# ai4ce/DiscoNet

Measured on AMD Instinct MI355X. Metric: scenes/sec (5-agent 256x256 BEV), higher is better.
Workload: dtype f16 hi+lo pair per value (32 bits; 22-bit significand for |x| >= 0.125, f16 exponent range, lo subnormal below: absolute floor 2^-25); conv products as split-f16 x3 MFMA, f32 accumulate; 1 GPU; DiscoNet det eval forward (--com disco), 5-agent, batch 4 per GPU, 256x256x13 BEV, no KD, sparse voxel lists -> dense -> enc -> DiscoGraph fusion -> dec -> cls/reg heads; agents=5, batch_per_gpu=4, conv_math=sp, launch=hipGraph replay, parallelism=scene-parallel x1 (no data-path collective)

## Files before the change

disconet_amd/csrc/build.py:

```python
import glob
import hashlib
import os
import subprocess
import sys
from concurrent.futures import ThreadPoolExecutor

HERE = os.path.dirname(os.path.abspath(__file__))
ROOT = os.path.dirname(os.path.dirname(HERE))
SOURCES = ["common.hip", "conv_mfma.hip", "conv_sp.hip", "conv_spq.hip", "voxel.hip", "warp.hip", "fuse_reduce.hip", "fuse_tail.hip", "fuse_mlp.hip", "agent_fuse.hip", "decode.hip", "detect.hip", "ap_match.hip", "assign.hip", "track.hip", "mot_eval.hip", "idf_eval.hip", "hota_eval.hip",
           "conv_wgrad.hip", "train_ops.hip", "seg_ops.hip", "seg_eval.hip", "render.hip", "lidar.hip"]
FLAGS = ["--offload-arch=gfx950", "-O3", "-std=c++17", "-fPIC", "-Wno-comment"]
LIB_PATH = os.path.join(os.path.dirname(HERE), "libdisconet_hip.so")


def tree_files():
    files = []
    for pat in ("*.hip", "*.inl", "*.h"):
        files += glob.glob(os.path.join(HERE, pat))
    files += glob.glob(os.path.join(ROOT, "include", "*.h"))
    return sorted(os.path.relpath(f, ROOT) for f in files)


def sources_present():
    return all(os.path.exists(os.path.join(HERE, s)) for s in SOURCES)


_HASH_CACHE = {}


def tree_hash(extra_flags=(), unit=None):
    try:
        stamp = (tuple(extra_flags), unit, tuple((rel,) + tuple(os.stat(os.path.join(ROOT, rel))[k] for k in (6, 8))
                                                  for rel in tree_files()))
    except OSError:
        stamp = None
    if stamp is not None and stamp in _HASH_CACHE:
        return _HASH_CACHE[stamp]
    h = hashlib.sha256()
    h.update(" ".join(FLAGS + list(extra_flags)).encode())
    for rel in tree_files():
        if unit is not None and rel.endswith(".hip") and os.path.basename(rel) != unit:
            continue
        h.update(b"\0" + rel.encode() + b"\0")
        with open(os.path.join(ROOT, rel), "rb") as f:
            h.update(f.read())
    if stamp is not None:
        _HASH_CACHE[stamp] = h.hexdigest()[:16]
    return h.hexdigest()[:16]


def built_id(path=None):
    import re
    path = path or LIB_PATH
    if not os.path.exists(path):
        return None
    with open(path, "rb") as f:
        m = re.search(rb"dn-build-id:([0-9a-f]{16})", f.read())
    return m.group(1).decode() if m else None


def needs_build():
    return built_id() != tree_hash()
# ... 62 lines not shown
```

disconet_amd/csrc/common.hip:

```cpp
#include "dn_internal.h"

namespace dn {
char* err_buf() {
  static thread_local char buf[512] = {0};
  return buf;
}
namespace {
typedef unsigned u32x4 __attribute__((ext_vector_type(4)));
__global__ void __launch_bounds__(256) zero_fill_kernel(unsigned char* p, size_t head, size_t vecs, size_t tail) {
  const size_t tid = blockIdx.x * (size_t)blockDim.x + threadIdx.x, stride = (size_t)gridDim.x * blockDim.x;
  if (tid < head) p[tid] = 0;
  u32x4* v = reinterpret_cast<u32x4*>(p + head);
  for (size_t i = tid; i < vecs; i += stride) v[i] = u32x4{0u, 0u, 0u, 0u};
  if (tid < tail) p[head + 16 * vecs + tid] = 0;
}
}

hipError_t zero_fill(void* ptr, size_t bytes, hipStream_t stream) {
  if (bytes == 0) return hipSuccess;
  unsigned char* p = static_cast<unsigned char*>(ptr);
  size_t head = (16 - (reinterpret_cast<size_t>(p) & 15)) & 15;
  if (head > bytes) head = bytes;
  const size_t vecs = (bytes - head) / 16, tail = bytes - head - 16 * vecs;
  const size_t want = (vecs + 255) / 256;
  const int blocks = (int)(want < 1 ? 1 : (want > 8192 ? 8192 : want));
  hipLaunchKernelGGL(zero_fill_kernel, dim3(blocks), dim3(256), 0, stream, p, head, vecs, tail);
  return hipGetLastError();
}
}

extern "C" int dn_version(void) { return 153; }

#ifndef DN_BUILD_ID
#error "build through disconet_amd/csrc/build.py (it passes -DDN_BUILD_ID)"
#endif
static const char dn_build_id_marker[] = "dn-build-id:" DN_BUILD_ID;
extern "C" const char* dn_build_id(void) { return dn_build_id_marker + 12; }

extern "C" int dn_sp_range_flags_async(unsigned* dst_device, int reset, void* stream) {
  DN_REQUIRE(dst_device != nullptr, "sp_range_flags_async: null destination");
  hipStream_t s = (hipStream_t)stream;
  if ((reset & 2) && dn::zero_fill(dst_device, sizeof(unsigned), s) != hipSuccess)
    return dn::fail(DN_ERR_LAUNCH, "sp_range_flags_async: zero fill of the destination failed");
  const bool clear = (reset & 1) != 0;
  dn::range_collect_conv_sp(dst_device, clear, s);
  dn::range_collect_conv_spq(dst_device, clear, s);
  dn::range_collect_fuse_mlp(dst_device, clear, s);
  dn::range_collect_conv_wgrad(dst_device, clear, s);
  return dn::check_launch("sp_range_collect_kernel");
}

extern "C" unsigned dn_sp_range_flags(int reset) {
  unsigned* d = nullptr;
  unsigned v = 0;
  if (hipDeviceSynchronize() != hipSuccess || hipMalloc((void**)&d, sizeof v) != hipSuccess) return 0x80000000u;
  bool ok = hipMemcpy(d, &v, sizeof v, hipMemcpyHostToDevice) == hipSuccess &&
            dn_sp_range_flags_async(d, reset ? 1 : 0, nullptr) == DN_OK &&
            hipMemcpy(&v, d, sizeof v, hipMemcpyDeviceToHost) == hipSuccess;
  (void)hipFree(d);
  return ok ? v : 0x80000000u;
}

extern "C" const char* dn_last_error(void) { return dn::err_buf(); }
```

disconet_amd/csrc/conv_sp.hip:

```cpp
#ifndef DN_PHASE_TIMING
#define DN_PHASE_TIMING 0
#endif
#ifndef DN_SP_ABL
#define DN_SP_ABL 0
#endif
#include "dn_internal.h"
#include "sp_layout.h"
#include "sp_device.h"
#include "sp_split.h"
#include <array>
#include <cstdlib>
#include <type_traits>
#include <utility>

#if DN_PHASE_TIMING
__device__ unsigned long long g_phase_cycles[8];
extern "C" int dn_sp_phase_cycles(unsigned long long* host8, int reset) {
  if (hipDeviceSynchronize() != hipSuccess) return -1;
  if (host8 && hipMemcpyFromSymbol(host8, HIP_SYMBOL(g_phase_cycles), sizeof(unsigned long long) * 8) != hipSuccess) return -1;
  if (reset) { unsigned long long z[8] = {0}; if (hipMemcpyToSymbol(HIP_SYMBOL(g_phase_cycles), z, sizeof z) != hipSuccess) return -1; }
  return 0;
}
#endif

// ... 1116 lines not shown
}

inline int out_dim(int in, int ksize, int stride) {
  const int pad = ksize / 2;
  return (in + 2 * pad - ksize) / stride + 1;
}
inline int cout_pad_of(int c_out) { return (c_out + 63) / 64 * 64; }
using sp::chunks_of;
int g_sp_upmode = -1;
inline int up_mode(const dn_conv_desc& d) {
  const int mode = g_sp_upmode >= 0 ? g_sp_upmode : 2;
  const bool ok = d.up0 == 1 && d.ksize == 3 && d.stride == 1 && d.c0 > 0 && d.c0 % 16 == 0 && d.h_in % 2 == 0 &&
                  d.w_in % 2 == 0;
  return ok ? (mode < 0 ? 0 : mode > 2 ? 2 : mode) : 0;
}
inline bool up_merged(const dn_conv_desc& d) { return up_mode(d) == 1; }
inline size_t packed_blocks(const dn_conv_desc& d);
inline int packed_chunks(const dn_conv_desc& d) { return (chunks_of(d.c0) + chunks_of(d.c1) + 3) / 4 * 4; }

int validate(const dn_conv_desc* d) {
  DN_REQUIRE(d != nullptr, "spconv: null descriptor");
  DN_REQUIRE(d->ksize == 1 || d->ksize == 3, "spconv: ksize %d unsupported (1 or 3)", d->ksize);
  DN_REQUIRE(d->stride == 1 || (d->stride == 2 && d->ksize == 3),
             "spconv: stride %d with ksize %d unsupported", d->stride, d->ksize);
  DN_REQUIRE(d->n_images > 0 && d->h_in > 0 && d->w_in > 0, "spconv: empty input");
  DN_REQUIRE(d->c0 > 0 && d->c1 >= 0 && d->c_out > 0, "spconv: bad channel counts");
  DN_REQUIRE(d->up0 == 0 || d->up0 == 1, "spconv: up0 must be 0 or 1");
  DN_REQUIRE(d->math != 3 || (d->ksize == 3 && d->stride == 1 && d->c1 == 0 && d->up0 == 0),
             "spconv: a hi-only source 0 (math = 3) needs a 3x3 stride-1 single-source layer");
  DN_REQUIRE(d->math != 4 || (d->ksize == 3 && d->stride == 1 && d->c1 == 0 && d->up0 == 0 && d->c0 <= 32),
             "spconv: a bit-grid source 0 (math = 4) needs a 3x3 stride-1 single-source layer of <= 32 channels");
  DN_REQUIRE(!d->up0 || (d->h_in % 2 == 0 && d->w_in % 2 == 0), "spconv: x2-upsampled source needs even h_in/w_in");
  DN_REQUIRE(d->c1 == 0 || (d->c0 % 16 == 0 && d->ksize == 3), "spconv: concat needs 3x3 and c0 %% 16 == 0 (c0 = %d)", d->c0);
  const size_t hs0 = d->up0 ? d->h_in / 2 : d->h_in, ws0 = d->up0 ? d->w_in / 2 : d->w_in;
  DN_REQUIRE(hs0 * ws0 * chunks_of(d->c0) * 64 < (1ull << 31) &&
                 (size_t)d->h_in * d->w_in * chunks_of(d->c1) * 64 < (1ull << 31),
             "spconv: one image must stay below 2 GiB");
  return DN_OK;
}

inline size_t packed_blocks(const dn_conv_desc& d) {
  const int nch = packed_chunks(d);
  if (up_mode(d) == 2) return dn::spq_packed_blocks(chunks_of(d.c0), nch);
  if (up_merged(d)) return (size_t)chunks_of(d.c0) * 12 + (size_t)(nch - chunks_of(d.c0)) * 9;
  return (size_t)nch * d.ksize * d.ksize;
}

enum SpCfgId { S3_256x64, S3_256x32, S3_128x64, S3_64x64, S3S2_128x64, S3S2_64x64, S1_256x64, S1_64x64,
               S3_256x64_T9, S3_512x64, S3_256x128, S1_256x64_C1, S3_256x32_ST, S3_64x64_T9, S3_128x64_T9,
               S3S2_64x64_T9, S3S2_128x64_T9, SP_CFG_COUNT };
enum SpForceId {
  FORCE_SPQ_BN32 = 20, FORCE_SPQ_BN64 = 21, FORCE_SPQ_DEEP = 22,
  FORCE_SPQ_ABL = 22,
  FORCE_TOOLS = 100,
  FORCE_ABL_256x64 = 100, FORCE_ABL_256x32 = 200,
  FORCE_ABL_64x64_T9 = 300,
  FORCE_ABL_S2_64x64 = 400,
};

template <int KS_, int STRIDE_, int TH_, int TW_, int BN_, int TG_, int CA_, int WAVES_M_, int WAVES_N_, int WTM_, int WTN_>
struct Geom {
  using G = Geom;
  static constexpr int KS = KS_, STRIDE = STRIDE_, TH = TH_, TW = TW_, BN = BN_, TG = TG_, CA = CA_, WAVES_M = WAVES_M_,
                       WAVES_N = WAVES_N_, WTM = WTM_, WTN = WTN_;
};
template <SpCfgId ID> struct Tile;
#define SP_TILE(id, bias_, deep_, ...) \
  template <> struct Tile<id> : __VA_ARGS__ { static constexpr float bias = bias_; static constexpr SpCfgId deep = deep_; }
SP_TILE(S3_256x64,      1.00f, S3_256x64_T9,   Geom<3, 1, 8,  32, 64,  3, 1, 4, 1, 2, 2>);
SP_TILE(S3_256x32,      1.15f, S3_256x32,      Geom<3, 1, 8,  32, 32,  3, 1, 4, 1, 2, 1>);
SP_TILE(S3_128x64,      1.10f, S3_128x64_T9,   Geom<3, 1, 8,  16, 64,  3, 1, 2, 2, 2, 1>);
SP_TILE(S3_64x64,       1.40f, S3_64x64_T9,    Geom<3, 1, 8,  8,  64,  3, 1, 2, 2, 1, 1>);
SP_TILE(S3S2_128x64,    1.45f, S3S2_128x64_T9, Geom<3, 2, 8,  16, 64,  3, 1, 2, 2, 2, 1>);
SP_TILE(S3S2_64x64,     1.00f, S3S2_64x64_T9,  Geom<3, 2, 8,  8,  64,  3, 1, 2, 2, 1, 1>);
SP_TILE(S1_256x64,      1.00f, S1_256x64,      Geom<1, 1, 8,  32, 64,  1, 2, 4, 1, 2, 2>);
SP_TILE(S1_64x64,       1.30f, S1_64x64,       Geom<1, 1, 8,  8,  64,  1, 4, 2, 2, 1, 1>);
SP_TILE(S3_256x64_T9,   1.f,   S3_256x64_T9,   Geom<3, 1, 8,  32, 64,  9, 1, 4, 1, 2, 2>);
SP_TILE(S3_512x64,      1.f,   S3_512x64,      Geom<3, 1, 16, 32, 64,  3, 1, 8, 1, 2, 2>);
SP_TILE(S3_256x128,     1.f,   S3_256x128,     Geom<3, 1, 8,  32, 128, 3, 1, 4, 2, 2, 2>);
SP_TILE(S1_256x64_C1,   1.2f,  S1_256x64_C1,   Geom<1, 1, 8,  32, 64,  1, 1, 4, 1, 2, 2>);
SP_TILE(S3_256x32_ST,   1.f,   S3_256x32_ST,   Tile<S3_256x32>::G);
SP_TILE(S3_64x64_T9,    1.f,   S3_64x64_T9,    Geom<3, 1, 8,  8,  64,  9, 1, 2, 2, 1, 1>);
SP_TILE(S3_128x64_T9,   1.f,   S3_128x64_T9,   Geom<3, 1, 8,  16, 64,  9, 1, 2, 2, 2, 1>);
SP_TILE(S3S2_64x64_T9,  1.f,   S3S2_64x64_T9,  Geom<3, 2, 8,  8,  64,  9, 1, 2, 2, 1, 1>);
SP_TILE(S3S2_128x64_T9, 1.f,   S3S2_128x64_T9, Geom<3, 2, 8,  16, 64,  9, 1, 2, 2, 2, 1>);
#undef SP_TILE

struct SpCfg { SpCfgId id; int th, tw, bn, ca; float bias; SpCfgId deep; };
template <int... I>
constexpr std::array<SpCfg, sizeof...(I)> sp_cfgs(std::integer_sequence<int, I...>) {
  return {{{(SpCfgId)I, Tile<(SpCfgId)I>::TH, Tile<(SpCfgId)I>::TW, Tile<(SpCfgId)I>::BN, Tile<(SpCfgId)I>::CA,
            Tile<(SpCfgId)I>::bias, Tile<(SpCfgId)I>::deep}...}};
}
constexpr std::array<SpCfg, SP_CFG_COUNT> kSpCfgs = sp_cfgs(std::make_integer_sequence<int, SP_CFG_COUNT>{});
int g_sp_force = -1;

SpCfg select_cfg(const dn_conv_desc& d, int kslices = 1, bool can_split = false) {
  const int ho = out_dim(d.h_in, d.ksize, d.stride), wo = out_dim(d.w_in, d.ksize, d.stride);
  static const SpCfgId c3[] = {S3_256x64, S3_256x32, S3_128x64, S3_64x64};
  static const SpCfgId c3s2[] = {S3S2_128x64, S3S2_64x64};
  static const SpCfgId c1[] = {S1_256x64, S1_64x64, S1_256x64_C1};
  static const SpCfgId c3up[] = {S3_256x32, S3_128x64};
  const bool upm = up_merged(d);
  static const SpCfgId c3ks[] = {S3_256x32, S3_128x64, S3_64x64};
  const bool ksl = kslices > 1 && d.ksize == 3 && !upm;
  const SpCfgId* cand = d.ksize == 1 ? c1 : (d.stride == 2 ? c3s2 : (upm ? c3up : (ksl ? c3ks : c3)));
// ... 369 lines not shown

extern "C" int dn_spconv2d_nhwc(const dn_conv_desc* d, const void* src0, const void* src1, const void* packed,
                                const float* scale, const float* shift, float* out_nhwc, int ld_nhwc, void* stream) {
  DN_REQUIRE(d && out_nhwc && ld_nhwc >= d->c_out && ld_nhwc % 4 == 0 && d->c_out % 4 == 0 &&
                 (reinterpret_cast<uintptr_t>(out_nhwc) & 15) == 0,
             "spconv nhwc: the fp32 NHWC output needs c_out %% 4 == 0, ld >= c_out, ld %% 4 == 0, 16-byte alignment");
  return spconv2d_impl(d, src0, src1, packed, scale, shift, nullptr, out_nhwc, ld_nhwc, stream);
}

inline bool ks_layer(const dn_conv_desc& d) { return d.ksize == 3 && d.math != 3 && d.math != 4 && up_mode(d) != 1; }

extern "C" int dn_spconv_ks_supported(const dn_conv_desc* d, int kslices) {
  if (validate(d) != DN_OK) return 0;
  if (kslices == 1) return 1;
  if (kslices != 2 && kslices != 4) return 0;
  return ks_layer(*d) && chunks_of(d->c0) + chunks_of(d->c1) >= kslices ? 1 : 0;
}

extern "C" size_t dn_spconv_workspace_bytes(const dn_conv_desc* d, int kslices) {
  if (validate(d) != DN_OK || kslices <= 1 || !ks_layer(*d)) return 0;
  const size_t ho = out_dim(d->h_in, d->ksize, d->stride), wo = out_dim(d->w_in, d->ksize, d->stride);
  return (size_t)kslices * d->n_images * ((ho + 7) / 8 * 8) * ((wo + 31) / 32 * 32) * ((d->c_out + 63) / 64 * 64) * sizeof(float);
}

extern "C" int dn_spconv2d_ks(const dn_conv_desc* d, int kslices, const void* src0, const void* src1, const void* packed,
                              const float* scale, const float* shift, void* out, float* out_nhwc, int ld_nhwc,
                              void* workspace, size_t workspace_bytes, void* stream) {
  DN_REQUIRE(kslices == 1 || kslices == 2 || kslices == 4, "spconv: kslices must be 1, 2 or 4 (got %d)", kslices);
  DN_REQUIRE(workspace == nullptr || (reinterpret_cast<uintptr_t>(workspace) & 15) == 0, "spconv: workspace must be 16-byte aligned");
  DN_REQUIRE(!out_nhwc || (d && ld_nhwc >= d->c_out && ld_nhwc % 4 == 0 && d->c_out % 4 == 0 &&
                           (reinterpret_cast<uintptr_t>(out_nhwc) & 15) == 0),
             "spconv: the fp32 NHWC output needs c_out %% 4 == 0, ld >= c_out, ld %% 4 == 0, 16-byte alignment");
  return spconv2d_impl(d, src0, src1, packed, scale, shift, out, out_nhwc, ld_nhwc, stream, kslices, workspace, workspace_bytes);
}

namespace {
int spconv2d_impl(const dn_conv_desc* d, const void* src0, const void* src1, const void* packed, const float* scale,
                  const float* shift, void* out, float* out_nhwc, int ld_nhwc, void* stream, int kslices,
                  void* workspace, size_t workspace_bytes) {
  if (int rc = validate(d)) return rc;
  DN_REQUIRE(src0 && packed && scale && shift && (out || out_nhwc), "spconv: null pointer");
  DN_REQUIRE(d->c1 == 0 || src1, "spconv: c1 > 0 but src1 is null");
  SpArgs a;
  if (int rc = fill_args(d, src0, src1, packed, scale, shift, out, a)) return rc;
  a.out_b = out_nhwc; a.ldo_b = ld_nhwc;
  DN_REQUIRE(!out_nhwc || g_sp_force < FORCE_TOOLS, "spconv dual: not with a forced tools configuration");
  hipStream_t s = (hipStream_t)stream;
  DN_REQUIRE(kslices == 1 || (ks_layer(*d) && a.c0g + a.c1g >= kslices),
             "spconv: %d K slices need a 3x3 layer of at least that many 16-channel chunks", kslices);
  if (up_mode(*d) == 2) {
    DN_REQUIRE(a.c1g == 0 || d->c0 % 16 == 0, "spconv: concat needs c0 %% 16 == 0");
    const int f = g_sp_force;
    const int bn = f == FORCE_SPQ_BN32 ? 32 : f == FORCE_SPQ_BN64 ? 64 : f == FORCE_SPQ_DEEP ? 33 :
                   (f > FORCE_SPQ_ABL && f <= FORCE_SPQ_ABL + 3) ? 100 + (f - FORCE_SPQ_ABL) : 0;
    return dn::spq_conv(d, src0, src1, packed, (size_t)a.wpk_bytes, scale, shift, out, a.cout_pad, bn, s, kslices,
                        (float*)workspace, workspace_bytes, out_nhwc, ld_nhwc);
  }
  if (kslices > 1) {
    a.ks.count = kslices;
    a.ks.partial = (float*)workspace;
    a.ks_ws_bytes = workspace_bytes;
    const SpCfg c = select_cfg(*d, kslices, workspace != nullptr && workspace_bytes > 0);
    const int rc = launch_form<KSliced, S3_256x32, S3_128x64, S3_64x64, S3S2_128x64, S3S2_64x64, S3_64x64_T9, S3_128x64_T9,
                               S3S2_64x64_T9, S3S2_128x64_T9>(c.id, a, *d, s);
    return rc != kNotListed ? rc : dn::fail(DN_ERR_UNSUPPORTED, "spconv: tile configuration %d has no K-sliced form", (int)c.id);
  }
  if (d->math == 3) {
    if (fits_stationary<HiOnlyStationary, S3_256x32>(*d, 0, 2)) return launch_form<HiOnlyStationary, S3_256x32>(a, *d, s);
    return launch_form<HiOnly, S3_256x32>(a, *d, s);
  }
  if (d->math == 4) {
    if (fits_stationary<BitGrid, S3_256x32>(*d, 0, 2)) return launch_form<BitGrid, S3_256x32>(a, *d, s);
    return dn::fail(DN_ERR_UNSUPPORTED, "spconv: a bit-grid source needs a layer whose weights fit the LDS (c_out <= 32)");
  }
  const SpCfg c = select_cfg(*d);
  if (up_merged(*d)) {
    const int rc = launch_form<RowMerged, S3_256x64, S3_256x32, S3_128x64>(c.id, a, *d, s);
    return rc != kNotListed ? rc : dn::fail(DN_ERR_UNSUPPORTED, "spconv: tile configuration %d has no row-merged form", (int)c.id);
  }
  if (d->ksize == 3 && d->stride == 1) {
    const int rc = launch_ablation<S3_64x64_T9, 1, 2, 3, 4, 5>(g_sp_force - FORCE_ABL_64x64_T9, a, *d, s);
    if (rc != kNotListed) return rc;
  }
#if DN_SP_ABL
  if (d->ksize == 3 && d->stride == 1) {
    int rc = launch_ablation<S3_256x64, 1, 2, 3, 4, 5>(g_sp_force - FORCE_ABL_256x64, a, *d, s);
    if (rc == kNotListed) rc = launch_ablation<S3_256x32, 1, 2, 3, 4, 5, 6, 7>(g_sp_force - FORCE_ABL_256x32, a, *d, s);
    if (rc != kNotListed) return rc;
  }
  if (d->ksize == 3 && d->stride == 2) {
    if (g_sp_force == FORCE_ABL_S2_64x64) return launch_form<Plain, S3S2_64x64>(a, *d, s);
    const int rc = launch_ablation<S3S2_64x64, 1, 2, 3, 4, 5, 7>(g_sp_force - FORCE_ABL_S2_64x64, a, *d, s);
    if (rc != kNotListed) return rc;
  }
#endif
  if (g_sp_force < 0 && c.id == S3_256x32 && fits_stationary<Stationary, S3_256x32>(*d, 0, 2))
    return launch_form<Stationary, S3_256x32>(a, *d, s);
  if (g_sp_force == S3_256x32_ST) return launch_form<Stationary, S3_256x32_ST>(a, *d, s);
  static const int b3_env = [] { const char* e = getenv("DN_SP_B3"); return e ? atoi(e) : 3; }();
  if (g_sp_force < 0 && c.id == S3S2_64x64 && (b3_env & 1)) return launch_form<ThreeStages, S3S2_64x64>(a, *d, s);
  if (g_sp_force < 0 && c.id == S3_64x64 && (b3_env & 2)) return launch_form<ThreeStages, S3_64x64>(a, *d, s);
  const int rc = launch_form<Plain, S3_256x64, S3_256x32, S3_128x64, S3_64x64, S3S2_128x64, S3S2_64x64, S1_256x64, S1_64x64,
                             S3_256x64_T9, S3_512x64, S3_256x128, S1_256x64_C1, S3_64x64_T9, S3_128x64_T9, S3S2_64x64_T9,
                             S3S2_128x64_T9>(c.id, a, *d, s);
  return rc != kNotListed ? rc : dn::fail(DN_ERR_UNSUPPORTED, "spconv: no tile configuration");
}
// ... 44 lines not shown
```

disconet_amd/csrc/conv_spq.hip:

```cpp
#ifndef DN_SP_ABL
#define DN_SP_ABL 0
#endif
#include "dn_internal.h"
#include "sp_layout.h"
#include "sp_device.h"
#include "sp_split.h"
#include <type_traits>

namespace {

constexpr int kCUs = 256;

constexpr int QTH = 8, QTW = 32, QPH = QTH + 2, QPW = QTW + 2, QHALF = QPW / 2, QPITCH = QPW, QNPIX = QPH * QPITCH;
constexpr int QNW = 4, QNT = QNW * 64;
constexpr int QA_PIECES = 4 * QNPIX;
constexpr int QA_INSTR = (QA_PIECES + 63) / 64;
constexpr int QA_IT = (QA_INSTR + QNW - 1) / QNW;
constexpr int QA_STAGE = QA_INSTR * 1024;
static_assert(QA_INSTR == 22 && QA_IT == 6, "patch stage: 22 instructions, waves 0 / 1 issue 6, waves 2 / 3 issue 5");

struct SpqArgs {
  const unsigned char* src0;
  const unsigned char* src1;
  const unsigned char* wpk;
// ... 636 lines not shown
    form.grid = (int)(work > resident ? resident : work); form.total_items = (int)work;
    form.n_whole = k.n_whole; form.n_split = k.n_split;
    form.fixup_grid = k.n_split ? (int)(k.n_split > 2 * kCUs ? 2 * kCUs : k.n_split) : 0;
    dn::g_sp_last_form = form;
    hipLaunchKernelGGL(kern, dim3((unsigned)(work > resident ? resident : work)), dim3(QNT), T::LDS_BYTES, stream, a);
    if (k.n_split) {
      k.fixup = 1;
      a.total_items = k.n_split;
      hipLaunchKernelGGL(kern, dim3((unsigned)(k.n_split > 2 * kCUs ? 2 * kCUs : k.n_split)), dim3(QNT), T::LDS_BYTES, stream, a);
    }
    return dn::check_launch("conv_spq_kernel (K slices)");
  }
  dim3 grid((unsigned)(total > resident ? resident : total));
  form.grid = (int)grid.x; form.total_items = (int)total; form.n_whole = (int)total;
  dn::g_sp_last_form = form;
  hipLaunchKernelGGL(kern, grid, dim3(QNT), T::LDS_BYTES, stream, a);
  return dn::check_launch("conv_spq_kernel");
}

}

namespace dn {

void range_collect_conv_spq(unsigned* dst, bool reset, hipStream_t s) { sp_range_collect_here(dst, reset, s); }

size_t spq_packed_blocks(int c0g, int nchunks) { return (size_t)c0g * 16 + (size_t)(nchunks - c0g) * 9; }

int spq_pack_weights(const float* weight_oihw, void* packed, int c_out, int c_in, int c0g, int cout_pad, int nchunks,
                     float wmul, hipStream_t stream) {
  hipLaunchKernelGGL(spq_pack_weights_kernel, dim3(2048), dim3(256), 0, stream, weight_oihw, (unsigned char*)packed, c_out,
                     c_in, c0g, cout_pad, nchunks, wmul);
  return check_launch("spq_pack_weights_kernel");
}

int spq_conv(const dn_conv_desc* d, const void* src0, const void* src1, const void* packed, size_t packed_bytes,
             const float* scale, const float* shift, void* out, int cout_pad, int bn, hipStream_t stream,
             int kslices, float* workspace, size_t workspace_bytes, float* out_nhwc, int ld_nhwc) {
  SpqArgs a;
  a.src0 = (const unsigned char*)src0; a.src1 = (const unsigned char*)src1; a.wpk = (const unsigned char*)packed;
  a.scale = scale; a.shift = shift; a.out = (unsigned char*)out;
  a.out_f32 = out_nhwc; a.ldo_f32 = ld_nhwc;
  a.n_images = d->n_images; a.h = d->h_in; a.w = d->w_in;
  a.c0g = (d->c0 + 15) / 16; a.c1g = (d->c1 + 15) / 16;
  a.c_out = d->c_out; a.cog = (d->c_out + 15) / 16; a.relu = d->relu;
  a.cout_pad = cout_pad; a.wpk_bytes = (int)packed_bytes;
  a.tiles_x = a.tiles_y = a.total_items = 0;
  a.ks = KSlices{workspace, kslices, 0, 0, 0, 0, 0, 0, 0, 0};
  if (kslices > 1) {
    const long tiles = (long)d->n_images * ((d->h_in + QTH - 1) / QTH) * ((d->w_in + QTW - 1) / QTW);
    const bool deep = tiles * ((d->c_out + 31) / 32) * kslices <= (long)kCUs;
    if (bn == 33 || (bn == 0 && deep)) return launch_spq<32, 1, 0, 1>(a, stream, workspace_bytes);
    return launch_spq<32, 0, 0, 1>(a, stream, workspace_bytes);
  }
  if (bn == 0) {
    const long tiles = (long)d->n_images * ((d->h_in + QTH - 1) / QTH) * ((d->w_in + QTW - 1) / QTW);
    bn = (d->c_out > 32 && tiles * ((d->c_out + 63) / 64) >= 4L * kCUs) ? 64 : 32;
    if (bn == 32 && tiles * ((d->c_out + 31) / 32) <= (long)kCUs) bn = 33;
  }
  if (bn == 64) return launch_spq<64>(a, stream);
  if (bn == 33) return launch_spq<32, 1>(a, stream);
#if DN_SP_ABL
  if (bn == 101) return launch_spq<32, 0, 1>(a, stream);
  if (bn == 102) return launch_spq<32, 0, 2>(a, stream);
  if (bn == 103) return launch_spq<32, 0, 3>(a, stream);
#endif
  return launch_spq<32>(a, stream);
}

}
```

disconet_amd/csrc/dn_internal.h:

```cpp
#pragma once
#include <hip/hip_runtime.h>
#include <cstdarg>
#include <cstdio>

#include "disconet_hip.h"

namespace dn {

char* err_buf();

inline int fail(int code, const char* fmt, ...) {
  va_list ap;
  va_start(ap, fmt);
  vsnprintf(err_buf(), 512, fmt, ap);
  va_end(ap);
  return code;
}

hipError_t zero_fill(void* ptr, size_t bytes, hipStream_t stream);

struct PerDeviceFlag {
  bool done[64] = {};
  bool& here() {
    int dev = 0;
    (void)hipGetDevice(&dev);
    return done[dev & 63];
  }
};

inline int static_lds_of(const void* kernel, PerDeviceFlag& flag, int* cache, int dynamic_most) {
  int dev = 0;
  (void)hipGetDevice(&dev);
  bool& ready = flag.done[dev & 63];
  if (!ready) {
    hipFuncAttributes attr;
    if (hipFuncGetAttributes(&attr, kernel) != hipSuccess) return -1;
    if (dynamic_most > 0 &&
        hipFuncSetAttribute(kernel, hipFuncAttributeMaxDynamicSharedMemorySize, dynamic_most) != hipSuccess)
      return -2;
    cache[dev & 63] = (int)attr.sharedSizeBytes;
    ready = true;
  }
  return cache[dev & 63];
}

inline int check_launch(const char* what) {
  hipError_t e = hipGetLastError();
  if (e != hipSuccess) return fail(DN_ERR_LAUNCH, "%s: %s", what, hipGetErrorString(e));
  return DN_OK;
}

size_t spq_packed_blocks(int c0g, int nchunks);
int spq_pack_weights(const float* weight_oihw, void* packed, int c_out, int c_in, int c0g, int cout_pad, int nchunks,
                     float wmul, hipStream_t stream);
int spq_conv(const dn_conv_desc* d, const void* src0, const void* src1, const void* packed, size_t packed_bytes,
             const float* scale, const float* shift, void* out, int cout_pad, int bn, hipStream_t stream,
             int kslices = 1, float* workspace = nullptr, size_t workspace_bytes = 0, float* out_nhwc = nullptr,
             int ld_nhwc = 0);

int fuse_mlp_agent_scores(const float* feat, const float* warped, int warped_fm, const int32_t* num_agent,
                          const dn_fuse_mlp_params* p, const float* w5, int batch, int agents, int hw, int c, int only_v2i,
                          int ego_first, int ego_count, float* partials, hipStream_t stream);

void range_collect_conv_sp(unsigned* dst, bool reset, hipStream_t stream);
void range_collect_conv_spq(unsigned* dst, bool reset, hipStream_t stream);
void range_collect_fuse_mlp(unsigned* dst, bool reset, hipStream_t stream);
void range_collect_conv_wgrad(unsigned* dst, bool reset, hipStream_t stream);
unsigned* sp_range_word();

struct SpLastForm {
  int family;
  int ks, stride, th, tw, bn, tg, ca, post, bstat, upm, ahi, ksl, nb, deep;
  int grid, total_items;
  int n_whole, n_split;
  int fixup_grid;
};
extern SpLastForm g_sp_last_form;

}

#define DN_REQUIRE(cond, ...) \
  do { if (!(cond)) return dn::fail(DN_ERR_ARG, __VA_ARGS__); } while (0)

#define DN_REQUIRE_EVAL_STEP(who, max_m, max_g)                                                                \
  DN_REQUIRE(rect, who ": null rect");                                                                         \
  DN_REQUIRE(id, who ": null id");                                                                             \
  DN_REQUIRE(count, who ": null count");                                                                       \
  DN_REQUIRE(gt_boxes, who ": null gt_boxes");                                                                 \
  DN_REQUIRE(gt_ids, who ": null gt_ids");                                                                     \
  DN_REQUIRE(gt_count, who ": null gt_count");                                                                 \
  DN_REQUIRE(state, who ": null state");                                                                       \
  DN_REQUIRE(m >= 1 && m <= (max_m), who ": M = %d track rows, must be in [1, %d]", m, (max_m));              \
  DN_REQUIRE(g >= 1 && g <= (max_g), who ": G = %d ground-truth rows, must be in [1, %d]", g, (max_g));       \
  DN_REQUIRE(std::isfinite(scale) && scale > 0, who ": scale = %g, must be finite and > 0", scale)
```

Baseline: 2328 scenes/s.

## Add wide 16x32 tile split-f16 upsample-concat conv kernel for narrow outputs

Adds a new quad-merged split-f16 MFMA conv kernel that uses a 16x32 spatial tile with 8 waves, double-buffered DMA staging of input patches and packed weights, and a persistent grid of one workgroup per CU. The dispatcher picks it by default (deep variant) when c_out <= 32 and there are enough tiles to cover the CUs at least twice. The aim is to raise MFMA utilisation and weight reuse for the decoder's narrow-output upsample+concat convolutions, which the smaller-tile path serves poorly. In exchange it uses a large LDS footprint (one workgroup per CU) and adds a separate code path that has to match the existing numerics.

```diff
diff --git a/disconet_amd/csrc/build.py b/disconet_amd/csrc/build.py
--- a/disconet_amd/csrc/build.py
+++ b/disconet_amd/csrc/build.py
@@ -7,7 +7,7 @@
 
 HERE = os.path.dirname(os.path.abspath(__file__))
 ROOT = os.path.dirname(os.path.dirname(HERE))
-SOURCES = ["common.hip", "conv_mfma.hip", "conv_sp.hip", "conv_spq.hip", "voxel.hip", "warp.hip", "fuse_reduce.hip", "fuse_tail.hip", "fuse_mlp.hip", "agent_fuse.hip", "decode.hip", "detect.hip", "ap_match.hip", "assign.hip", "track.hip", "mot_eval.hip", "idf_eval.hip", "hota_eval.hip",
+SOURCES = ["common.hip", "conv_mfma.hip", "conv_sp.hip", "conv_spq.hip", "conv_spq_wide.hip", "voxel.hip", "warp.hip", "fuse_reduce.hip", "fuse_tail.hip", "fuse_mlp.hip", "agent_fuse.hip", "decode.hip", "detect.hip", "ap_match.hip", "assign.hip", "track.hip", "mot_eval.hip", "idf_eval.hip", "hota_eval.hip",
            "conv_wgrad.hip", "train_ops.hip", "seg_ops.hip", "seg_eval.hip", "render.hip", "lidar.hip"]
 FLAGS = ["--offload-arch=gfx950", "-O3", "-std=c++17", "-fPIC", "-Wno-comment"]
 LIB_PATH = os.path.join(os.path.dirname(HERE), "libdisconet_hip.so")
diff --git a/disconet_amd/csrc/common.hip b/disconet_amd/csrc/common.hip
--- a/disconet_amd/csrc/common.hip
+++ b/disconet_amd/csrc/common.hip
@@ -29,7 +29,7 @@
 }
 }
 
-extern "C" int dn_version(void) { return 153; }
+extern "C" int dn_version(void) { return 154; }
 
 #ifndef DN_BUILD_ID
 #error "build through disconet_amd/csrc/build.py (it passes -DDN_BUILD_ID)"
diff --git a/disconet_amd/csrc/conv_sp.hip b/disconet_amd/csrc/conv_sp.hip
--- a/disconet_amd/csrc/conv_sp.hip
+++ b/disconet_amd/csrc/conv_sp.hip
@@ -1192,6 +1192,7 @@
 enum SpForceId {
   FORCE_SPQ_BN32 = 20, FORCE_SPQ_BN64 = 21, FORCE_SPQ_DEEP = 22,
   FORCE_SPQ_ABL = 22,
+  FORCE_SPQ_WIDE = 26, FORCE_SPQ_WIDE_DEEP = 27,
   FORCE_TOOLS = 100,
   FORCE_ABL_256x64 = 100, FORCE_ABL_256x32 = 200,
   FORCE_ABL_64x64_T9 = 300,
@@ -1667,6 +1668,7 @@
     DN_REQUIRE(a.c1g == 0 || d->c0 % 16 == 0, "spconv: concat needs c0 %% 16 == 0");
     const int f = g_sp_force;
     const int bn = f == FORCE_SPQ_BN32 ? 32 : f == FORCE_SPQ_BN64 ? 64 : f == FORCE_SPQ_DEEP ? 33 :
+                   f == FORCE_SPQ_WIDE ? 34 : f == FORCE_SPQ_WIDE_DEEP ? 35 :
                    (f > FORCE_SPQ_ABL && f <= FORCE_SPQ_ABL + 3) ? 100 + (f - FORCE_SPQ_ABL) : 0;
     return dn::spq_conv(d, src0, src1, packed, (size_t)a.wpk_bytes, scale, shift, out, a.cout_pad, bn, s, kslices,
                         (float*)workspace, workspace_bytes, out_nhwc, ld_nhwc);
diff --git a/disconet_amd/csrc/conv_spq.hip b/disconet_amd/csrc/conv_spq.hip
--- a/disconet_amd/csrc/conv_spq.hip
+++ b/disconet_amd/csrc/conv_spq.hip
@@ -712,6 +712,9 @@
     if (bn == 33 || (bn == 0 && deep)) return launch_spq<32, 1, 0, 1>(a, stream, workspace_bytes);
     return launch_spq<32, 0, 0, 1>(a, stream, workspace_bytes);
   }
+  if (bn == 0 && d->c_out <= 32 && spq_wide_tiles(d) >= 2L * kCUs) bn = 35;
+  if (bn == 34 || bn == 35)
+    return spq_wide_conv(d, src0, src1, packed, packed_bytes, scale, shift, out, cout_pad, bn == 35, stream, out_nhwc, ld_nhwc);
   if (bn == 0) {
     const long tiles = (long)d->n_images * ((d->h_in + QTH - 1) / QTH) * ((d->w_in + QTW - 1) / QTW);
     bn = (d->c_out > 32 && tiles * ((d->c_out + 63) / 64) >= 4L * kCUs) ? 64 : 32;
diff --git a/disconet_amd/csrc/conv_spq_wide.hip b/disconet_amd/csrc/conv_spq_wide.hip
--- /dev/null
+++ b/disconet_amd/csrc/conv_spq_wide.hip
@@ -0,0 +1,471 @@
+#include "dn_internal.h"
+#include "sp_layout.h"
+#include "sp_device.h"
+#include "sp_split.h"
+#include <type_traits>
+
+namespace {
+
+constexpr int kCUs = 256;
+
+constexpr int WTH = 16, WTW = 32, WPH = WTH + 2, WPW = WTW + 2, WHALF = WPW / 2, WPITCH = WPW, WNPIX = WPH * WPITCH;
+constexpr int WNW = 8, WNT = WNW * 64, BN = 32;
+constexpr int WA_PIECES = 4 * WNPIX;
+constexpr int WA_INSTR = (WA_PIECES + 63) / 64;
+constexpr int WA_IT = (WA_INSTR + WNW - 1) / WNW;
+constexpr int WA_LAST = WA_INSTR - (WA_IT - 1) * WNW;
+constexpr int WA_STAGE = WA_INSTR * 1024;
+static_assert(WA_INSTR == 39 && WA_IT == 5 && WA_LAST == 7, "patch stage: 39 instructions, waves 0..6 issue 5, wave 7 issues 4");
+static_assert(WPH <= 255 && WPW <= 255, "piece_map packs row and column into bytes");
+
+struct SpqWideArgs {
+  const unsigned char* src0;
+  const unsigned char* src1;
+  const unsigned char* wpk;
+  const float* scale;
+  const float* shift;
+  unsigned char* out;
+  float* out_f32;
+  unsigned* range_word;
+  int ldo_f32;
+  int n_images, h, w;
+  int c0g, c1g;
+  int c_out, cog, relu;
+  int tiles_x, tiles_y, total_items;
+  int cout_pad, wpk_bytes;
+  float rcp_tx, rcp_ty;
+};
+
+struct WTile {
+  int img, oy0, ox0;
+};
+
+template <int DEEP>
+struct SpqWideTile {
+  static constexpr int TGQ = DEEP ? 4 : 2;
+  static constexpr int NS0 = 4 / TGQ;
+  static constexpr int TG1 = DEEP ? 9 : 3;
+  static constexpr int NS1 = 9 / TG1;
+  static constexpr int BLK = 4 * BN * 16;
+  static constexpr int B_PIECES0 = TGQ * 4 * 4 * BN;
+  static constexpr int B_PIECES1 = TG1 * 4 * BN;
+  static constexpr int B_IT0 = (B_PIECES0 + WNT - 1) / WNT;
+  static constexpr int B_IT1 = (B_PIECES1 + WNT - 1) / WNT;
+  static_assert(B_IT1 <= B_IT0, "the source-0 step is the larger one");
+  static constexpr int WB_STAGE = B_IT0 * WNT * 16;
+  static constexpr int AFF_BYTES = WNW * 2 * 64 * 4;
+  static constexpr int LDS_BYTES = 2 * WA_STAGE + 2 * WB_STAGE + AFF_BYTES;
+  static_assert(LDS_BYTES == (DEEP ? 149504 : 116736) && LDS_BYTES <= 160 * 1024, "one workgroup per CU");
+};
+
+__device__ inline void note_range_at(unsigned* word, float amax, bool nan_seen) {
+  if (amax > 16384.f) atomicOr(word, amax >= 65504.f ? 3u : 2u);
+  if (nan_seen) atomicOr(word, 4u);
+}
+
+template <int DEEP>
+__global__ void __launch_bounds__(WNT, 2) conv_spq_kernel_wide(const SpqWideArgs a) {
+  using T = SpqWideTile<DEEP>;
+  constexpr int TGQ = T::TGQ, NS0 = T::NS0, NS1 = T::NS1, BLK = T::BLK, WB_STAGE = T::WB_STAGE;
+  extern __shared__ __attribute__((aligned(16))) unsigned char smem[];
+  constexpr int OFF_B = 2 * WA_STAGE;
+
+  const int tid = threadIdx.x;
+  const int lane = tid & 63;
+  const int wave = tid >> 6;
+  const int li = lane & 31, lh = lane >> 5;
+  const int py = wave & 1, px = (wave >> 1) & 1, half = wave >> 2;
+
+  const int G = gridDim.x;
+  const int spatial_items = a.n_images * a.tiles_y * a.tiles_x;
+  const int sp_full = spatial_items & ~7;
+  auto decode = [&](int item) {
+    WTile tc;
+    int spi = item < sp_full ? (item & 7) * (sp_full >> 3) + (item >> 3) : item;
+    int tx, ty;
+    spi = fdivmod(spi, a.tiles_x, a.rcp_tx, tx);
+    tc.img = fdivmod(spi, a.tiles_y, a.rcp_ty, ty);
+    tc.ox0 = tx * WTW;
+    tc.oy0 = ty * WTH;
+    return tc;
+  };
+  const int nchunks = a.c0g + a.c1g;
+
+  const int rsel = sp::in_g2(li) ? 1 : 0, kcol = sp::rank16(li);
+  int prow[2], pcol;
+  pcol = px + 2 * kcol;
+  auto colpos = [](int e) { return (e & 1) * WHALF + (e >> 1); };
+  int a_b1[2][3];
+  int a_b0[2][2][2];
+#pragma unroll
+  for (int wm = 0; wm < 2; ++wm) {
+    prow[wm] = py + 4 * wm + 2 * rsel + 8 * half;
+#pragma unroll
+    for (int dx = 0; dx < 3; ++dx) a_b1[wm][dx] = (lh * WNPIX + prow[wm] * WPITCH + colpos(px + dx) + kcol) * 16;
+#pragma unroll
+    for (int b = 0; b < 2; ++b)
+#pragma unroll
+      for (int am = 0; am < 2; ++am)
+        a_b0[wm][b][am] = (lh * WNPIX + (prow[wm] + am + (py & am)) * WPITCH + colpos(px + b + (px & b)) + kcol) * 16;
+  }
+  const int b_off = (lh * BN + li) * 16;
+  const int b_offq = b_off + (wave & 3) * BLK;
+
+  f32x16 acc[2];
+  float amax = 0.f;
+  bool nan_seen = false;
+
+  constexpr unsigned OOB = 0xFFFFFFFFu;
+  const int hs0 = a.h >> 1, ws0 = a.w >> 1;
+  const unsigned plane0 = (unsigned)(hs0 * ws0) * 16u, plane1 = (unsigned)(a.h * a.w) * 16u;
+  const size_t img0_bytes = (size_t)a.c0g * 4 * plane0, img1_bytes = (size_t)a.c1g * 4 * plane1;
+  auto rsrc0 = __builtin_amdgcn_make_buffer_rsrc(const_cast<unsigned char*>(a.src0), 0, 0, 0x00020000);
+  auto rsrc1 = rsrc0;
+  const auto rsrcw = __builtin_amdgcn_make_buffer_rsrc(const_cast<unsigned char*>(a.wpk), 0, a.wpk_bytes, 0x00020000);
+  unsigned voff_a[WA_IT], voff_b[T::B_IT0];
+
+  auto opaque = [](int v) {
+    asm volatile("" : "+v"(v));
+    return v;
+  };
+  unsigned piece_map[WA_IT];
+#pragma unroll
+  for (int it = 0; it < WA_IT; ++it) {
+    const int piece = (it * WNW + wave) * 64 + lane;
+    const int cq = piece / WNPIX, pp = piece % WNPIX;
+    const int r = pp / WPITCH, pos = pp % WPITCH;
+    const int cc = pos < WHALF ? 2 * pos : 2 * (pos - WHALF) + 1;
+    piece_map[it] = (unsigned)r | ((unsigned)cc << 8) | ((unsigned)cq << 16) | (piece < WA_PIECES ? 0x80000000u : 0u);
+  }
+  auto setup_voff_a = [&](const WTile& tc, bool from1) {
+    const int iy0 = tc.oy0 - 1, ix0 = tc.ox0 - 1;
+    const unsigned plane = from1 ? plane1 : plane0;
+    const int ws = from1 ? a.w : ws0;
+#pragma unroll
+    for (int it = 0; it < WA_IT; ++it) {
+      unsigned pm = piece_map[it];
+      asm volatile("" : "+v"(pm));
+      const int r = pm & 0xff, cc = (pm >> 8) & 0xff, cq = (pm >> 16) & 0xff;
+      const int iy = iy0 + r, ix = ix0 + cc;
+      const bool ok = (int)pm < 0 && iy >= 0 && iy < a.h && ix >= 0 && ix < a.w;
+      const int sy = from1 ? iy : (iy >> 1), sx = from1 ? ix : (ix >> 1);
+      voff_a[it] = ok ? (unsigned)cq * plane + (unsigned)(sy * ws + sx) * 16u : OOB;
+    }
+  };
+  {
+    const int t = opaque(tid);
+#pragma unroll
+    for (int it = 0; it < T::B_IT0; ++it) {
+      const int piece = (it * WNW + (t >> 6)) * 64 + (t & 63);
+      const int blk = piece / (4 * BN), q = (piece / BN) % 4, nn = piece % BN;
+      voff_b[it] = (unsigned)(((blk * 4 + q) * a.cout_pad + nn) * 16);
+    }
+  }
+  auto setup_rsrc = [&](const WTile& tc) {
+    rsrc0 = __builtin_amdgcn_make_buffer_rsrc(const_cast<unsigned char*>(a.src0 + tc.img * img0_bytes), 0,
+                                              (int)img0_bytes, 0x00020000);
+    rsrc1 = __builtin_amdgcn_make_buffer_rsrc(const_cast<unsigned char*>(a.c1g ? a.src1 + tc.img * img1_bytes : a.src0),
+                                              0, a.c1g ? (int)img1_bytes : 0, 0x00020000);
+  };
+  auto issue_a = [&](int g, int sa) {
+    const bool from1 = g >= a.c0g;
+    const int soff = from1 ? (g - a.c0g) * 4 * (int)plane1 : g * 4 * (int)plane0;
+    unsigned char* base = smem + sa * WA_STAGE + wave * 1024;
+#pragma unroll
+    for (int it = 0; it < WA_IT; ++it) {
+      if (it == WA_IT - 1 && wave >= WA_LAST) break;
+      if (from1)
+        dma16(rsrc1, base + it * WNW * 1024, voff_a[it], soff);
+      else
+        dma16(rsrc0, base + it * WNW * 1024, voff_a[it], soff);
+    }
+  };
+  auto issue_b = [&](int g, int st, int sb) {
+    const bool from1 = g >= a.c0g;
+    const int blk = from1 ? a.c0g * 16 + (g - a.c0g) * 9 + st * T::TG1 : g * 16 + st * (TGQ * 4);
+    const int soff = blk * 4 * a.cout_pad * 16;
+    unsigned char* base = smem + OFF_B + sb * WB_STAGE + wave * 1024;
+#pragma unroll
+    for (int it = 0; it < T::B_IT0; ++it)
+      if (!from1 || it < T::B_IT1) dma16(rsrcw, base + it * WNW * 1024, voff_b[it], soff);
+  };
+
+  struct Frags {
+    half8 ah[2], al[2], bh, bl;
+  };
+  auto mma = [&](const Frags& f) {
+#pragma unroll
+    for (int wm = 0; wm < 2; ++wm) acc[wm] = __builtin_amdgcn_mfma_f32_32x32x16_f16(f.bl, f.ah[wm], acc[wm], 0, 0, 0);
+#pragma unroll
+    for (int wm = 0; wm < 2; ++wm) acc[wm] = __builtin_amdgcn_mfma_f32_32x32x16_f16(f.bh, f.al[wm], acc[wm], 0, 0, 0);
+#pragma unroll
+    for (int wm = 0; wm < 2; ++wm) acc[wm] = __builtin_amdgcn_mfma_f32_32x32x16_f16(f.bh, f.ah[wm], acc[wm], 0, 0, 0);
+  };
+  auto compute1 = [&](auto st_c, const unsigned char* As, const unsigned char* Bs) {
+    constexpr int DY = decltype(st_c)::value;
+    Frags f[2];
+    auto load = [&](auto u_c) {
+      constexpr int u = decltype(u_c)::value;
+      Frags& d = f[u & 1];
+#pragma unroll
+      for (int wm = 0; wm < 2; ++wm) {
+        d.ah[wm] = *reinterpret_cast<const half8*>(As + a_b1[wm][u] + DY * WPITCH * 16);
+        d.al[wm] = *reinterpret_cast<const half8*>(As + a_b1[wm][u] + DY * WPITCH * 16 + 2 * WNPIX * 16);
+      }
+      d.bh = *reinterpret_cast<const half8*>(Bs + b_off + u * BLK);
+      d.bl = *reinterpret_cast<const half8*>(Bs + b_off + u * BLK + 2 * BN * 16);
+    };
+    load(std::integral_constant<int, 0>{});
+    load(std::integral_constant<int, 1>{});
+    __builtin_amdgcn_sched_barrier(0);
+    mma(f[0]);
+    __builtin_amdgcn_sched_barrier(0);
+    load(std::integral_constant<int, 2>{});
+    __builtin_amdgcn_sched_barrier(0);
+    mma(f[1]);
+    __builtin_amdgcn_sched_barrier(0);
+    mma(f[0]);
+    __builtin_amdgcn_sched_barrier(0);
+  };
+  auto compute0 = [&](auto st_c, const unsigned char* As, const unsigned char* Bs) {
+    constexpr int ST = decltype(st_c)::value;
+    Frags f[2];
+    auto load = [&](auto u_c) {
+      constexpr int u = decltype(u_c)::value;
+      constexpr int t = ST * TGQ + u, am = t >> 1, b = t & 1;
+      Frags& d = f[u & 1];
+#pragma unroll
+      for (int wm = 0; wm < 2; ++wm) {
+        d.ah[wm] = *reinterpret_cast<const half8*>(As + a_b0[wm][b][am]);
+        d.al[wm] = *reinterpret_cast<const half8*>(As + a_b0[wm][b][am] + 2 * WNPIX * 16);
+      }
+      d.bh = *reinterpret_cast<const half8*>(Bs + b_offq + u * 4 * BLK);
+      d.bl = *reinterpret_cast<const half8*>(Bs + b_offq + u * 4 * BLK + 2 * BN * 16);
+    };
+    load(std::integral_constant<int, 0>{});
+    load(std::integral_constant<int, 1>{});
+    __builtin_amdgcn_sched_barrier(0);
+    mma(f[0]);
+    __builtin_amdgcn_sched_barrier(0);
+    if constexpr (TGQ == 4) {
+      load(std::integral_constant<int, 2>{});
+      __builtin_amdgcn_sched_barrier(0);
+      mma(f[1]);
+      __builtin_amdgcn_sched_barrier(0);
+      load(std::integral_constant<int, 3>{});
+      __builtin_amdgcn_sched_barrier(0);
+      mma(f[0]);
+      __builtin_amdgcn_sched_barrier(0);
+    }
+    mma(f[1]);
+    __builtin_amdgcn_sched_barrier(0);
+  };
+
+  float* aff_s = reinterpret_cast<float*>(smem + 2 * WA_STAGE + 2 * WB_STAGE) + wave * 128;
+  if (lane < BN) {
+    const int ci = min(lane, a.c_out - 1);
+    aff_s[lane] = lane < a.c_out ? a.scale[ci] : 0.f;
+    aff_s[64 + lane] = lane < a.c_out ? a.shift[ci] : 0.f;
+  }
+  auto epilogue = [&](const WTile& tc) {
+    const int plane = a.h * a.w * 16;
+    const int img_bytes = a.cog * 4 * plane;
+    const auto rsrc_o = __builtin_amdgcn_make_buffer_rsrc(a.out + (size_t)tc.img * img_bytes, 0, img_bytes, 0x00020000);
+    const float lo_clamp = a.relu ? 0.f : -65504.f;
+    if (a.out_f32 != nullptr) {
+      const float floor_v = a.relu ? 0.f : -__builtin_inff();
+#pragma unroll
+      for (int wm = 0; wm < 2; ++wm) {
+        const int oy = tc.oy0 + prow[wm], ox = tc.ox0 + pcol;
+        const bool inside = oy < a.h && ox < a.w;
+        float* orow = a.out_f32 + (((size_t)tc.img * a.h + oy) * a.w + ox) * a.ldo_f32;
+#pragma unroll
+        for (int g = 0; g < 4; ++g) {
+          const int co = 8 * g + 4 * lh;
+          const f32x4 sc = *reinterpret_cast<const f32x4*>(aff_s + 8 * g + 4 * lh);
+          const f32x4 sh = *reinterpret_cast<const f32x4*>(aff_s + 64 + 8 * g + 4 * lh);
+          f32x4 v = affine4(quad_of(acc[wm], g), sc, sh);
+          nan_seen |= !(fabsf(v[0]) <= 3.4028235e38f) | !(fabsf(v[1]) <= 3.4028235e38f) | !(fabsf(v[2]) <= 3.4028235e38f) |
+                      !(fabsf(v[3]) <= 3.4028235e38f);
+#pragma unroll
+          for (int e = 0; e < 4; ++e) v[e] = fmaxf(v[e], floor_v);
+          if (inside && co < a.c_out) *reinterpret_cast<f32x4*>(orow + co) = v;
+        }
+      }
+      if (a.out == nullptr) return;
+    }
+#pragma unroll
+    for (int wm = 0; wm < 2; ++wm) {
+      const int oy = tc.oy0 + prow[wm], ox = tc.ox0 + pcol;
+      const bool inside = oy < a.h && ox < a.w;
+      const int voff = inside ? (oy * a.w + ox) * 16 + lh * plane : (int)0x80000000;
+      u32x2 hi[4], lo[4];
+#pragma unroll
+      for (int g = 0; g < 4; ++g) {
+        const f32x4 sc = *reinterpret_cast<const f32x4*>(aff_s + 8 * g + 4 * lh);
+        const f32x4 sh = *reinterpret_cast<const f32x4*>(aff_s + 64 + 8 * g + 4 * lh);
+        const f32x4 v = affine4(quad_of(acc[wm], g), sc, sh);
+        split4(v, hi[g], lo[g], amax, lo_clamp);
+      }
+#pragma unroll
+      for (int m = 0; m < 2; ++m) {
+        const u32x4 ph = gather_octet(hi[2 * m], hi[2 * m + 1]);
+        const u32x4 pl = gather_octet(lo[2 * m], lo[2 * m + 1]);
+        if (m < a.cog) {
+          __builtin_amdgcn_raw_buffer_store_b128(ph, rsrc_o, voff + m * 4 * plane, 0, 0);
+          __builtin_amdgcn_raw_buffer_store_b128(pl, rsrc_o, voff + (m * 4 + 2) * plane, 0, 0);
+        }
+      }
+    }
+  };
+
+  int item = blockIdx.x;
+  if (item >= a.total_items) return;
+  WTile cur = decode(item);
+  setup_rsrc(cur);
+  setup_voff_a(cur, a.c0g == 0);
+  issue_b(0, 0, 0);
+  issue_a(0, 0);
+  int sa = 0, sb = 0;
+  bool a_pending = true;
+  int st_out = 0;
+
+  while (true) {
+#pragma unroll
+    for (int wm = 0; wm < 2; ++wm)
+#pragma unroll
+      for (int r = 0; r < 16; ++r) acc[wm][r] = 0.f;
+    const bool has_next = item + G < a.total_items;
+    WTile nxt = cur;
+    if (has_next) nxt = decode(item + G);
+
+    for (int g = 0; g < nchunks; ++g) {
+      const bool last_g = g + 1 == nchunks;
+      auto step = [&](auto st_c, auto kind_c) {
+        constexpr int ST = decltype(st_c)::value;
+        constexpr bool SRC1 = decltype(kind_c)::value;
+        constexpr int NSG = SRC1 ? NS1 : NS0;
+        if (ST == 1 && a_pending) {
+          if (wave < WA_LAST) wait_vm<WA_IT>(); else wait_vm<WA_IT - 1>();
+        } else if (ST == 0 && g == 0 && st_out == 8) {
+          wait_vm<8>();
+        } else if (ST == 0 && g == 0 && st_out == 4) {
+          wait_vm<4>();
+        } else {
+          wait_vm0();
+        }
+        __builtin_amdgcn_s_barrier();
+        asm volatile("" ::: "memory");
+        if (ST + 1 < NSG) {
+          issue_b(g, ST + 1, sb ^ 1);
+        } else if (!last_g) {
+          issue_b(g + 1, 0, sb ^ 1);
+        } else if (has_next) {
+          issue_b(0, 0, sb ^ 1);
+        }
+        if (ST == 0) {
+          a_pending = true;
+          if (!last_g) {
+            if (g + 1 == a.c0g) setup_voff_a(cur, true);
+            issue_a(g + 1, sa ^ 1);
+          } else if (has_next) {
+            setup_rsrc(nxt);
+            setup_voff_a(nxt, a.c0g == 0);
+            issue_a(0, sa ^ 1);
+          } else {
+            a_pending = false;
+          }
+        }
+        if constexpr (SRC1 && NS1 == 1) {
+          compute1(std::integral_constant<int, 0>{}, smem + sa * WA_STAGE, smem + OFF_B + sb * WB_STAGE);
+          compute1(std::integral_constant<int, 1>{}, smem + sa * WA_STAGE, smem + OFF_B + sb * WB_STAGE + 3 * BLK);
+          compute1(std::integral_constant<int, 2>{}, smem + sa * WA_STAGE, smem + OFF_B + sb * WB_STAGE + 6 * BLK);
+        } else if constexpr (SRC1)
+          compute1(st_c, smem + sa * WA_STAGE, smem + OFF_B + sb * WB_STAGE);
+        else
+          compute0(st_c, smem + sa * WA_STAGE, smem + OFF_B + sb * WB_STAGE);
+        sb ^= 1;
+      };
+      if (g < a.c0g) {
+        step(std::integral_constant<int, 0>{}, std::false_type{});
+        if constexpr (NS0 == 2) step(std::integral_constant<int, 1>{}, std::false_type{});
+      } else {
+        step(std::integral_constant<int, 0>{}, std::true_type{});
+        if constexpr (NS1 == 3) {
+          step(std::integral_constant<int, 1>{}, std::true_type{});
+          step(std::integral_constant<int, 2>{}, std::true_type{});
+        }
+      }
+      sa ^= 1;
+    }
+    epilogue(cur);
+    st_out = a.out_f32 == nullptr ? 4 * min(a.cog, 2) : 0;
+    note_range_at(a.range_word, amax, nan_seen);
+    if (!has_next) break;
+    item += G;
+    cur = nxt;
+  }
+}
+
+template <int DEEP>
+int launch_spq_wide(SpqWideArgs& a, hipStream_t stream) {
+  using T = SpqWideTile<DEEP>;
+  auto kern = conv_spq_kernel_wide<DEEP>;
+  static dn::PerDeviceFlag attr_flag;
+  static unsigned* range_word[64];
+  int dev = 0;
+  (void)hipGetDevice(&dev);
+  bool& attr_set = attr_flag.here();
+  if (!attr_set) {
+    hipError_t e = hipFuncSetAttribute(reinterpret_cast<const void*>(kern), hipFuncAttributeMaxDynamicSharedMemorySize,
+                                       (int)T::LDS_BYTES);
+    if (e != hipSuccess)
+      return dn::fail(DN_ERR_LAUNCH, "spconv (quad-merged, 16 x 32): hipFuncSetAttribute(%d B LDS): %s", (int)T::LDS_BYTES,
+                      hipGetErrorString(e));
+    range_word[dev & 63] = dn::sp_range_word();
+    DN_REQUIRE(range_word[dev & 63], "spconv (quad-merged, 16 x 32): the range word of the split-f16 engine is not addressable");
+    attr_set = true;
+  }
+  a.range_word = range_word[dev & 63];
+  a.tiles_x = (a.w + WTW - 1) / WTW;
+  a.tiles_y = (a.h + WTH - 1) / WTH;
+  const long total = (long)a.n_images * a.tiles_y * a.tiles_x;
+  DN_REQUIRE(total < (1L << 22), "spconv (quad-merged, 16 x 32): too many tiles (%ld)", total);
+  DN_REQUIRE((long)a.h * a.w * 16 * 4 * a.cog < (1L << 31), "spconv (quad-merged, 16 x 32): one output image exceeds 2 GiB");
+  a.total_items = (int)total;
+  a.rcp_tx = 1.0f / (float)a.tiles_x; a.rcp_ty = 1.0f / (float)a.tiles_y;
+  const long resident = kCUs;
+  dim3 grid((unsigned)(total > resident ? resident : total));
+  dn::g_sp_last_form = dn::SpLastForm{3, 3, 1, WTH, WTW, BN, 0, 1, 0, 0, 2, 0, 0, 0, DEEP, (int)grid.x, (int)total, (int)total, 0, 0};
+  hipLaunchKernelGGL(kern, grid, dim3(WNT), T::LDS_BYTES, stream, a);
+  return dn::check_launch("conv_spq_kernel_wide");
+}
+
+}
+
+namespace dn {
+
+long spq_wide_tiles(const dn_conv_desc* d) {
+  return (long)d->n_images * ((d->h_in + WTH - 1) / WTH) * ((d->w_in + WTW - 1) / WTW);
+}
+
+int spq_wide_conv(const dn_conv_desc* d, const void* src0, const void* src1, const void* packed, size_t packed_bytes,
+                  const float* scale, const float* shift, void* out, int cout_pad, int deep, hipStream_t stream,
+                  float* out_nhwc, int ld_nhwc) {
+  DN_REQUIRE(d->c_out >= 1 && d->c_out <= BN, "spconv (quad-merged, 16 x 32): c_out %d, the tile holds one block of %d channels",
+             d->c_out, BN);
+  DN_REQUIRE(d->c0 >= 1, "spconv (quad-merged, 16 x 32): no upsampled source");
+  SpqWideArgs a;
+  a.src0 = (const unsigned char*)src0; a.src1 = (const unsigned char*)src1; a.wpk = (const unsigned char*)packed;
+  a.scale = scale; a.shift = shift; a.out = (unsigned char*)out;
+  a.out_f32 = out_nhwc; a.ldo_f32 = ld_nhwc; a.range_word = nullptr;
+  a.n_images = d->n_images; a.h = d->h_in; a.w = d->w_in;
+  a.c0g = (d->c0 + 15) / 16; a.c1g = (d->c1 + 15) / 16;
+  a.c_out = d->c_out; a.cog = (d->c_out + 15) / 16; a.relu = d->relu;
+  a.cout_pad = cout_pad; a.wpk_bytes = (int)packed_bytes;
+  a.tiles_x = a.tiles_y = a.total_items = 0;
+  a.rcp_tx = a.rcp_ty = 0.f;
+  return deep ? launch_spq_wide<1>(a, stream) : launch_spq_wide<0>(a, stream);
+}
+
+}
diff --git a/disconet_amd/csrc/dn_internal.h b/disconet_amd/csrc/dn_internal.h
--- a/disconet_amd/csrc/dn_internal.h
+++ b/disconet_amd/csrc/dn_internal.h
@@ -58,6 +58,11 @@
              int kslices = 1, float* workspace = nullptr, size_t workspace_bytes = 0, float* out_nhwc = nullptr,
              int ld_nhwc = 0);
 
+long spq_wide_tiles(const dn_conv_desc* d);
+int spq_wide_conv(const dn_conv_desc* d, const void* src0, const void* src1, const void* packed, size_t packed_bytes,
+                  const float* scale, const float* shift, void* out, int cout_pad, int deep, hipStream_t stream,
+                  float* out_nhwc, int ld_nhwc);
+
 int fuse_mlp_agent_scores(const float* feat, const float* warped, int warped_fm, const int32_t* num_agent,
                           const dn_fuse_mlp_params* p, const float* w5, int batch, int agents, int hw, int c, int only_v2i,
                           int ego_first, int ego_count, float* partials, hipStream_t stream);
```

Result: no change. 2336 scenes/s, median of 6 (+0.4%).
